# cmhungsteve/TA3N

Measured on NVIDIA H100. Metric: video-clips/sec fwd+bwd (B=256,T=5,D=2048), higher is better.
Workload: dtype tf32x3

## Files before the change

ta3n_b200/csrc/gemm_wgmma.cuh:

```cuda
#pragma once

#include <cuda.h>
#include <stdlib.h>

#include <algorithm>
#include <cmath>
#include <functional>
#include <map>
#include <tuple>

#include "seg_gemm.cuh"

namespace ta3n {

constexpr int TC_BM = 128, TC_BN = 128, TC_BK = 32;
constexpr int TC_THREADS = 288;
constexpr int TC_CONSUMER_WARPS = 8;
constexpr int TC_A_BYTES = TC_BM * TC_BK * 4;
constexpr int TC_B_BYTES = TC_BN * TC_BK * 4;
constexpr int TC_STAGE_BYTES = TC_A_BYTES + TC_B_BYTES;
constexpr int TC_STAGES = 4;
constexpr int tc_smem_bytes(int stages) { return stages * TC_STAGE_BYTES + 1024; }
constexpr int TC_ACC_LD = TC_BN + 4;
constexpr int TC_ACC_BYTES = TC_BM * TC_ACC_LD * 4;
static_assert(TC_ACC_BYTES <= TC_STAGES * TC_STAGE_BYTES, "the per-launch kernel reuses its operand ring");
#ifndef TA3N_MAX_MAPS
#define TA3N_MAX_MAPS 64
#endif
constexpr int kMaxMaps = TA3N_MAX_MAPS;

struct alignas(64) TcMaps {
  CUtensorMap m[kMaxMaps];
};
struct TcSegMaps {
  unsigned char a[kMaxSegs];
  unsigned char b[kMaxSegs];
};

__device__ __forceinline__ uint32_t smem_u32(const void* p) { return (uint32_t)__cvta_generic_to_shared(p); }

__device__ __forceinline__ void mbar_init(uint64_t* bar, uint32_t count) {
  asm volatile("mbarrier.init.shared::cta.b64 [%0], %1;" ::"r"(smem_u32(bar)), "r"(count) : "memory");
}
__device__ __forceinline__ void mbar_expect_tx(uint64_t* bar, uint32_t bytes) {
  asm volatile("mbarrier.arrive.expect_tx.shared::cta.b64 _, [%0], %1;" ::"r"(smem_u32(bar)), "r"(bytes) : "memory");
}
__device__ __forceinline__ void mbar_wait(uint64_t* bar, uint32_t parity) {
  const uint32_t addr = smem_u32(bar);
  uint32_t done;
  do {
    asm volatile(
        "{\n\t.reg .pred p;\n\t"
        "mbarrier.try_wait.parity.shared::cta.b64 p, [%1], %2;\n\t"
        "selp.u32 %0, 1, 0, p;\n\t}"
        : "=r"(done)
        : "r"(addr), "r"(parity)
        : "memory");
  } while (!done);
}
__device__ __forceinline__ void mbar_arrive(uint64_t* bar) {
  asm volatile("mbarrier.arrive.shared::cta.b64 _, [%0];" ::"r"(smem_u32(bar)) : "memory");
}
__device__ __forceinline__ void fence_barrier_init() { asm volatile("fence.mbarrier_init.release.cluster;" ::: "memory"); }
__device__ __forceinline__ void fence_proxy_async() { asm volatile("fence.proxy.async.shared::cta;" ::: "memory"); }
__device__ __forceinline__ void consumer_sync() { asm volatile("bar.sync 1, 256;" ::: "memory"); }

__device__ __forceinline__ void tma_load_2d(void* smem_dst, const CUtensorMap* map, uint64_t* bar, int c0, int c1) {
  asm volatile(
      "cp.async.bulk.tensor.2d.shared::cluster.global.mbarrier::complete_tx::bytes [%0], [%1, {%3, %4}], [%2];"
      ::"r"(smem_u32(smem_dst)), "l"(map), "r"(smem_u32(bar)), "r"(c0), "r"(c1)
      : "memory");
// ... 86 lines not shown
  for (int i = 0; i < 4; ++i) r[i] = lds4(base + mnmaj_chunk(4 * kq + i, mq));
}
__device__ __forceinline__ void tc_prep_store(const uint32_t base, const int t, const float4 (&r)[4]) {
  int mq, kq;
  tc_prep_blk(t, &mq, &kq);
#pragma unroll
  for (int i = 0; i < 4; ++i)
    sts4(base + kmaj_chunk(4 * mq + i, kq), make_float4(f4_at(r[0], i), f4_at(r[1], i), f4_at(r[2], i), f4_at(r[3], i)));
}
__device__ __forceinline__ void tc_prep_stage(const uint32_t a_base, const uint32_t b_base, const bool a_kmaj,
                                              const bool b_kmaj) {
  if (a_kmaj && b_kmaj) return;
  const int t = threadIdx.x;
  float4 ra[4], rb[4];
  if (!a_kmaj) tc_prep_load(a_base, t, ra);
  if (!b_kmaj) tc_prep_load(b_base, t, rb);
  consumer_sync();
  if (!a_kmaj) tc_prep_store(a_base, t, ra);
  if (!b_kmaj) tc_prep_store(b_base, t, rb);
  fence_proxy_async();
  consumer_sync();
}

__device__ __forceinline__ void tc_store_acc(float* acc, const float (&d)[64], const int t) {
  const int lane = t & 31;
  const int row0 = (t >> 7) * 64 + ((t >> 5) & 3) * 16 + (lane >> 2);
#pragma unroll
  for (int j = 0; j < 16; ++j)
#pragma unroll
    for (int h = 0; h < 2; ++h)
      *reinterpret_cast<float2*>(acc + (row0 + 8 * h) * TC_ACC_LD + 8 * j + 2 * (lane & 3)) =
          make_float2(d[4 * j + 2 * h], d[4 * j + 2 * h + 1]);
}
__device__ __forceinline__ void acc_ld_32(const float* acc, int row, int col0, float* v) {
  const float* p = acc + row * TC_ACC_LD + col0;
#pragma unroll
  for (int j = 0; j < 32; j += 4) {
    const float4 q = *reinterpret_cast<const float4*>(p + j);
    v[j] = q.x;
    v[j + 1] = q.y;
    v[j + 2] = q.z;
    v[j + 3] = q.w;
  }
}

struct TcShared {
  uint64_t full_bar[4];
  uint64_t empty_bar[4];
};

template <int STAGES>
__device__ __forceinline__ void tc_pipe_init(TcShared* sh) {
  for (int s = 0; s < STAGES; ++s) {
    mbar_init(&sh->full_bar[s], 1);
    mbar_init(&sh->empty_bar[s], TC_CONSUMER_WARPS);
  }
  fence_barrier_init();
}

enum : int { TILE_FINAL = 0, TILE_PARTIAL = 1 };

template <int STAGES, int STAGE_BYTES = TC_STAGE_BYTES>
__device__ __forceinline__ void tc_produce(const TileCtx& ctx, const CUtensorMap* __restrict__ maps, const bool a_kmaj,
                                           const bool b_kmaj, const int pad_flags, const int m0, const int n0,
                                           const int c_begin, const int n_iter, uint8_t* smem, TcShared* sh,
                                           const uint32_t slabs) {
  const Group& g = ctx.g;
  int seg = 0, k0 = 0;
  {
    int skip = c_begin;
    while (seg < g.seg_count) {
      const int nch = (ctx.seg[seg].len + TC_BK - 1) / TC_BK;
      if (skip < nch) {
        k0 = skip * TC_BK;
        break;
      }
      skip -= nch;
      ++seg;
// ... 35 lines not shown

template <int STAGES>
__device__ __forceinline__ void tc_consume(const bool a_kmaj, const bool b_kmaj, const int n_iter, uint8_t* smem,
                                           TcShared* sh, float (&d)[64]) {
  const int wg = threadIdx.x >> 7, lane = threadIdx.x & 31;
#pragma unroll
  for (int j = 0; j < 64; ++j) d[j] = 0.f;
  int prev = -1;
  for (int it = 0; it < n_iter; ++it) {
    const uint32_t gl = (uint32_t)it;
    const int stage = (int)(gl % STAGES);
    mbar_wait(&sh->full_bar[stage], (gl / STAGES) & 1u);
    const uint32_t a_base = smem_u32(smem + stage * TC_STAGE_BYTES);
    const uint32_t b_base = a_base + TC_A_BYTES;
    tc_prep_stage(a_base, b_base, a_kmaj, b_kmaj);
    wgmma_fence();
#pragma unroll
    for (int ks = 0; ks < TC_BK / 8; ++ks) wgmma_tf32(d, wgmma_desc(a_base + wg * 64 * 128, ks), wgmma_desc(b_base, ks));
    wgmma_commit();
    wgmma_wait<1>();
    if (prev >= 0) {
      __syncwarp();
      if (lane == 0) mbar_arrive(&sh->empty_bar[prev]);
    }
    prev = stage;
  }
  wgmma_wait<0>();
  if (prev >= 0) {
    __syncwarp();
    if (lane == 0) mbar_arrive(&sh->empty_bar[prev]);
  }
}

template <int kEpiWarps>
__device__ __forceinline__ void tc_epilogue(const TileCtx& ctx, const int m0, const int n0, const int split,
                                            const int n_iter, const int mode, const float* acc, const int ew) {
  const int lane = threadIdx.x & 31;
  const int lq = ew & 3;
  const Group e = ctx.g;
  const int m = m0 + lq * 32 + lane;
  const bool split_out = mode == TILE_PARTIAL;
  float* const obase = split_out ? e.partial + (size_t)split * e.M * e.N : e.C;
  const int ldo = split_out ? e.N : e.ldc;
  constexpr int kColChunks = (TC_BN / 32) * 4 / kEpiWarps;
  const int c0 = (ew / 4) * kColChunks;
#pragma unroll 1
  for (int c = c0; c < c0 + kColChunks; ++c) {
    float v[32];
    if (n_iter > 0) {
      acc_ld_32(acc, lq * 32 + lane, c * 32, v);
    } else {
#pragma unroll
      for (int j = 0; j < 32; ++j) v[j] = 0.f;
    }
    const int nb = n0 + c * 32;
    if (m < e.M && nb < e.N) {
      float* orow = obase + (size_t)m * ldo + nb;
      const int nvalid = min(32, e.N - nb);
      if (!split_out) {
        TA3N_EPI_DISPATCH(e.flags, { epilogue_row32<EPI_F>(e, m, nb, nvalid, v); })
      }
      if (nb + 32 <= e.N && ((reinterpret_cast<uintptr_t>(orow) & 15u) == 0)) {
#pragma unroll
        for (int j = 0; j < 32; j += 4)
          *reinterpret_cast<float4*>(orow + j) = make_float4(v[j], v[j + 1], v[j + 2], v[j + 3]);
      } else {
#pragma unroll
        for (int j = 0; j < 32; ++j)
          if (nb + j < e.N) orow[j] = v[j];
      }
    }
  }
}

__device__ __forceinline__ void tc_chunk_range(const TileCtx& ctx, int split, int* c_begin, int* n_iter) {
  const Group& g = ctx.g;
  int total_chunks = 0;
  for (int s = 0; s < g.seg_count; ++s) total_chunks += (ctx.seg[s].len + TC_BK - 1) / TC_BK;
  const int cps = (total_chunks + g.ksplit - 1) / g.ksplit;
  *c_begin = split * cps;
  *n_iter = max(0, min(total_chunks, *c_begin + cps) - *c_begin);
}

__device__ __forceinline__ void tc_decode(const TileCtx& ctx, const int tile, int* split, int* m0, int* n0) {
  const Group& g = ctx.g;
  int local = tile - g.tile_begin;
  const int per_split = g.tiles_m * g.tiles_n;
  *split = local / per_split;
  local -= *split * per_split;
  *m0 = (local / g.tiles_n) * TC_BM;
  *n0 = (local % g.tiles_n) * TC_BN;
}

template <bool A_KMAJ, bool B_KMAJ>
__global__ void __launch_bounds__(TC_THREADS, 1)
seg_gemm_tc_kernel(const __grid_constant__ GemmTable tab, const __grid_constant__ TcMaps maps,
                   const __grid_constant__ TcSegMaps segmaps, const int first_wave) {
  extern __shared__ uint8_t tc_smem_raw[];
  __shared__ __align__(8) TcShared sh;
  uint8_t* smem = reinterpret_cast<uint8_t*>((reinterpret_cast<uintptr_t>(tc_smem_raw) + 1023) & ~uintptr_t(1023));
  const int warp = threadIdx.x >> 5, lane = threadIdx.x & 31;

  __shared__ TileCtx ctx;
  int tile = blockIdx.x;
  if (tile >= first_wave) tile = tab.total_tiles - 1 - (tile - first_wave);
  load_tile_ctx(tab, tile, &ctx, segmaps.a, segmaps.b);
  int split, m0, n0, c_begin, n_iter;
  tc_decode(ctx, tile, &split, &m0, &n0);
  tc_chunk_range(ctx, split, &c_begin, &n_iter);

  if (warp == TC_CONSUMER_WARPS && lane == 0) tc_pipe_init<TC_STAGES>(&sh);
  __syncthreads();
  pdl_wait();

  const int mode = ctx.g.ksplit > 1 ? TILE_PARTIAL : TILE_FINAL;
  if (warp == TC_CONSUMER_WARPS) {
    if (lane == 0 && n_iter > 0)
      tc_produce<TC_STAGES>(ctx, maps.m, A_KMAJ, B_KMAJ, tab.pad_, m0, n0, c_begin, n_iter, smem, &sh, 0u);
  } else {
    float d[64];
    tc_consume<TC_STAGES>(A_KMAJ, B_KMAJ, n_iter, smem, &sh, d);
    consumer_sync();
    float* acc = reinterpret_cast<float*>(smem);
    tc_store_acc(acc, d, threadIdx.x);
    consumer_sync();
    tc_epilogue<TC_CONSUMER_WARPS>(ctx, m0, n0, split, n_iter, mode, acc, warp);
  }
}

constexpr int X3_THREADS = 384;
constexpr int X3_SPLIT_WARPS = 3;
constexpr int X3_SPLIT_THREADS = 32 * X3_SPLIT_WARPS;
constexpr int X3_PRODUCER_REGS = 40, X3_CONSUMER_REGS = 232;
static_assert(128 * X3_PRODUCER_REGS + 256 * X3_CONSUMER_REGS <= X3_THREADS * 168,
              "setmaxnreg budget exceeds the registers of one CTA");
constexpr int X3_STAGES = 4;
constexpr int X3_STAGE_BYTES = TC_STAGE_BYTES + TC_B_BYTES;
constexpr int X3_CHUNK = 8;
static_assert(X3_CHUNK % 2 == 0, "the A fragment register sets alternate by slab within a chunk");
constexpr int x3_smem_bytes() { return X3_STAGES * X3_STAGE_BYTES + 1024; }

constexpr int kX3MaxCtas = 144;
constexpr int kX3MaxTasks = 1024;
struct X3Sched {
  int listed;
  unsigned short off[kX3MaxCtas + 1];
  unsigned short task[kX3MaxTasks];
};
static_assert(sizeof(GemmTable) + sizeof(TcMaps) + sizeof(TcSegMaps) + sizeof(X3Sched) + 256 <= 32764,
              "kernel parameters of the precise kernel exceed the 32 KB limit");

struct X3Slot {
  TileCtx ctx;
  int split, m0, n0, c_begin, n_iter;
};
constexpr int X3_SLOT_READERS = TC_CONSUMER_WARPS + 3;

__device__ __forceinline__ int x3_task(const X3Sched& sched, const int k) {
  return sched.listed ? (int)sched.task[sched.off[blockIdx.x] + k] : (int)(blockIdx.x + k * gridDim.x);
// ... 176 lines not shown
        }
      } else {
        x0 = epilogue_t<F>(g, m, n, x0);
        if (two) x1 = epilogue_t<F>(g, m, n + 1, x1);
      }
      x3_st2(C + (size_t)m * ldc + n, x0, x1, vec, two);
    }
  }
}

__device__ __forceinline__ void x3_finish(const X3Slot& sl, const float (&v)[64]) {
  const Group& g = sl.ctx.g;
  const int warp = threadIdx.x >> 5, lane = threadIdx.x & 31;
  const int m0 = sl.m0 + (warp >> 2) * 64 + (warp & 3) * 16 + (lane >> 2), n0 = sl.n0 + 2 * (lane & 3);
  if (g.ksplit > 1) {
    const int M = g.M, N = g.N;
    float* const part = g.partial + (size_t)sl.split * M * N;
    const bool vec = (N % 2) == 0;
#pragma unroll
    for (int h = 0; h < 2; ++h)
#pragma unroll
      for (int j = 0; j < 16; ++j) {
        const int m = m0 + 8 * h, n = n0 + 8 * j;
        if (m < M && n < N) x3_st2(part + (size_t)m * N + n, v[4 * j + 2 * h], v[4 * j + 2 * h + 1], vec, n + 1 < N);
      }
    return;
  }
  TA3N_EPI_DISPATCH(g.flags, { x3_epilogue<EPI_F>(g, m0, n0, v); })
}

template <bool A_KMAJ, bool B_KMAJ>
__global__ void __launch_bounds__(X3_THREADS, 1)
seg_gemm_tc_x3_kernel(const __grid_constant__ GemmTable tab, const __grid_constant__ TcMaps maps,
                      const __grid_constant__ TcSegMaps segmaps, const __grid_constant__ X3Sched sched) {
  extern __shared__ uint8_t tc_smem_raw[];
  __shared__ __align__(8) TcShared sh;
  __shared__ __align__(8) uint64_t ready_bar[X3_STAGES];
  __shared__ __align__(8) uint64_t slot_full[2], slot_empty[2];
  __shared__ X3Slot slots[2];
  uint8_t* smem = reinterpret_cast<uint8_t*>((reinterpret_cast<uintptr_t>(tc_smem_raw) + 1023) & ~uintptr_t(1023));
  const int warp = threadIdx.x >> 5, lane = threadIdx.x & 31;
  const int n_tasks = sched.listed ? sched.off[blockIdx.x + 1] - sched.off[blockIdx.x]
                                   : (tab.total_tiles - (int)blockIdx.x + (int)gridDim.x - 1) / (int)gridDim.x;

  if (warp == TC_CONSUMER_WARPS) {
    if (lane == 0) {
      for (int s = 0; s < X3_STAGES; ++s) mbar_init(&ready_bar[s], X3_SPLIT_WARPS);
      for (int s = 0; s < 2; ++s) {
        mbar_init(&slot_full[s], 1);
        mbar_init(&slot_empty[s], X3_SLOT_READERS);
      }
      tc_pipe_init<X3_STAGES>(&sh);
    }
    __syncwarp();
    x3_stage(tab, segmaps, x3_task(sched, 0), &slots[0]);
    if (lane == 0) mbar_arrive(&slot_full[0]);
  }
  __syncthreads();
  pdl_wait();

  if (warp >= TC_CONSUMER_WARPS) {
    setmaxnreg_dec<X3_PRODUCER_REGS>();
    uint32_t slabs = 0;
    if (warp == TC_CONSUMER_WARPS) {
      for (int k = 0; k < n_tasks; ++k) {
        const int s = k & 1;
        if (k > 0) {
          mbar_wait(&slot_empty[s], ((uint32_t)(k >> 1) & 1u) ^ 1u);
          x3_stage(tab, segmaps, x3_task(sched, k), &slots[s]);
          if (lane == 0) mbar_arrive(&slot_full[s]);
        }
        const X3Slot& sl = slots[s];
        if (lane == 0 && sl.n_iter > 0)
          tc_produce<X3_STAGES, X3_STAGE_BYTES>(sl.ctx, maps.m, A_KMAJ, B_KMAJ, tab.pad_, sl.m0, sl.n0, sl.c_begin,
                                                sl.n_iter, smem, &sh, slabs);
        __syncwarp();
        slabs += (uint32_t)sl.n_iter;
      }
    } else {
      const int t = threadIdx.x - 32 * (TC_CONSUMER_WARPS + 1);
      for (int k = 0; k < n_tasks; ++k) {
        const int s = k & 1;
        mbar_wait(&slot_full[s], (uint32_t)(k >> 1) & 1u);
        const int n_iter = slots[s].n_iter;
        __syncwarp();
        if (lane == 0) mbar_arrive(&slot_empty[s]);
        for (int it = 0; it < n_iter; ++it) {
          const uint32_t gl = slabs + (uint32_t)it;
          const int stage = (int)(gl % X3_STAGES);
          mbar_wait(&sh.full_bar[stage], (gl / X3_STAGES) & 1u);
          const uint32_t b_raw = smem_u32(smem + stage * X3_STAGE_BYTES) + TC_A_BYTES;
          x3_split_b<B_KMAJ>(b_raw, b_raw + TC_B_BYTES, t);
          fence_proxy_async();
          __syncwarp();
          if (lane == 0) mbar_arrive(&ready_bar[stage]);
        }
        slabs += (uint32_t)n_iter;
      }
    }
  } else {
    setmaxnreg_inc<X3_CONSUMER_REGS>();
    const int r0 = (warp >> 2) * 64 + (warp & 3) * 16 + (lane >> 2);
    const uint32_t off0 = x3_a_thread_off<A_KMAJ>(r0, lane & 3), off1 = x3_a_thread_off<A_KMAJ>(r0 + 8, lane & 3);
    uint32_t slabs = 0;
    for (int k = 0; k < n_tasks; ++k) {
      const int s = k & 1;
      mbar_wait(&slot_full[s], (uint32_t)(k >> 1) & 1u);
      const int n_iter = slots[s].n_iter;
      float d[64], sum[64];
#pragma unroll
      for (int j = 0; j < 64; ++j) d[j] = sum[j] = 0.f;
      uint32_t hi[2][16], lo[2][16];
      int prev = -1;
      for (int c0 = 0; c0 < n_iter; c0 += X3_CHUNK) {
        const int c1 = min(n_iter, c0 + X3_CHUNK);
        for (int it = c0; it < c1; it += 2) {
          x3_consume_slab<A_KMAJ>(slabs + (uint32_t)it, smem, &sh, ready_bar, off0, off1, hi[0], lo[0], d, prev);
          if (it + 1 < c1)
            x3_consume_slab<A_KMAJ>(slabs + (uint32_t)(it + 1), smem, &sh, ready_bar, off0, off1, hi[1], lo[1], d, prev);
        }
        wgmma_wait<0>();
        __syncwarp();
        if (lane == 0) mbar_arrive(&sh.empty_bar[prev]);
        prev = -1;
#pragma unroll
        for (int j = 0; j < 64; ++j) {
          sum[j] += d[j];
          d[j] = 0.f;
        }
      }
      slabs += (uint32_t)n_iter;
      x3_finish(slots[s], sum);
      __syncwarp();
      if (lane == 0) mbar_arrive(&slot_empty[s]);
    }
  }
}

typedef CUresult (*PFN_encodeTiled)(CUtensorMap*, CUtensorMapDataType, cuuint32_t, void*, const cuuint64_t*,
                                    const cuuint64_t*, const cuuint32_t*, const cuuint32_t*, CUtensorMapInterleave,
                                    CUtensorMapSwizzle, CUtensorMapL2promotion, CUtensorMapFloatOOBfill);

inline PFN_encodeTiled encode_fn() {
  static PFN_encodeTiled fn = []() -> PFN_encodeTiled {
    void* p = nullptr;
    cudaDriverEntryPointQueryResult q;
    if (cudaGetDriverEntryPoint("cuTensorMapEncodeTiled", &p, cudaEnableDefault, &q) != cudaSuccess) return nullptr;
    if (q != cudaDriverEntryPointSuccess) return nullptr;
    return reinterpret_cast<PFN_encodeTiled>(p);
  }();
  return fn;
}

struct DeviceInfo {
  int sm_count = 0;
  bool configured[4] = {false, false, false, false};
  bool x3_configured[4] = {false, false, false, false};
  bool eval_configured = false;
};
inline std::mutex& device_mu() {
  static std::mutex mu;
  return mu;
}
inline DeviceInfo* device_info() {
  static std::map<int, DeviceInfo> devs;
  int dev = 0;
  if (cudaGetDevice(&dev) != cudaSuccess) return nullptr;
  DeviceInfo& d = devs[dev];
// ... 65 lines not shown
inline bool tc_group_ok(const GemmPlan& plan, const Group& g) {
  if (plan.load_flags != 0) return false;
  if ((long)g.M * g.N < 64L * 64L) return false;
  if (g.seg_count > kMaxSegs) return false;
  std::map<MapKey, int> maps;
  for (int i = 0; i < g.seg_count; ++i) {
    const Seg& s = plan.segs[g.seg_begin + i];
    if (!tc_operand_ok(s.A, s.lda) || !tc_operand_ok(s.B, s.ldb) || s.len <= 0) return false;
    MapKey ka, kb;
    tc_seg_keys(s, g, plan.a_kmaj, plan.b_kmaj, false, false, &ka, &kb);
    maps[ka] = maps[kb] = 0;
  }
  return (int)maps.size() <= kMaxMaps;
}

template <bool A_KMAJ, bool B_KMAJ>
inline int tc_launch_one(const GemmTable& tab, const TcMaps& maps, const TcSegMaps& sm, cudaStream_t stream,
                         const char* label) {
  constexpr int slot = (A_KMAJ ? 0 : 1) + (B_KMAJ ? 0 : 2);
  int first_wave = 132;
  {
    std::lock_guard<std::mutex> lock(device_mu());
    DeviceInfo* d = device_info();
    if (!d) return fail(TA3N_ERR_CUDA, "cudaGetDevice failed");
    if (!d->configured[slot]) {
      TA3N_CUDA(cudaFuncSetAttribute(seg_gemm_tc_kernel<A_KMAJ, B_KMAJ>, cudaFuncAttributeMaxDynamicSharedMemorySize,
                                     tc_smem_bytes(TC_STAGES)));
      d->configured[slot] = true;
    }
    first_wave = d->sm_count;
  }
  pre_launch(label, stream);
  launch_kernel(seg_gemm_tc_kernel<A_KMAJ, B_KMAJ>, tab.total_tiles, TC_THREADS, tc_smem_bytes(TC_STAGES), stream, tab,
                maps, sm, first_wave);
  return after_launch();
}

template <bool A_KMAJ, bool B_KMAJ>
inline int tc_launch_x3(const GemmTable& tab, const TcMaps& maps, const TcSegMaps& sm, const X3Sched& sched, int grid,
                        cudaStream_t stream, const char* label) {
  constexpr int slot = (A_KMAJ ? 0 : 1) + (B_KMAJ ? 0 : 2);
  {
    std::lock_guard<std::mutex> lock(device_mu());
    DeviceInfo* d = device_info();
    if (!d) return fail(TA3N_ERR_CUDA, "cudaGetDevice failed");
    if (!d->x3_configured[slot]) {
      TA3N_CUDA(cudaFuncSetAttribute(seg_gemm_tc_x3_kernel<A_KMAJ, B_KMAJ>, cudaFuncAttributeMaxDynamicSharedMemorySize,
                                     x3_smem_bytes()));
      d->x3_configured[slot] = true;
    }
  }
  pre_launch(label, stream);
  launch_kernel(seg_gemm_tc_x3_kernel<A_KMAJ, B_KMAJ>, grid, X3_THREADS, x3_smem_bytes(), stream, tab, maps, sm, sched);
  return after_launch();
}

inline GemmPlan sub_plan(const GemmPlan& plan, const std::vector<int>& idx) {
  GemmPlan out;
  out.a_kmaj = plan.a_kmaj;
  out.b_kmaj = plan.b_kmaj;
  out.load_flags = plan.load_flags;
  out.label = plan.label;
  for (int i : idx) {
    Group g = plan.groups[i];
    const int b = g.seg_begin;
    g.seg_begin = (int)out.segs.size();
    for (int k = 0; k < g.seg_count; ++k) out.segs.push_back(plan.segs[b + k]);
    out.groups.push_back(g);
  }
  return out;
}

inline void tc_rank3_flags(const GemmPlan& plan, bool* a3d, bool* b3d) {
  *a3d = !plan.a_kmaj;
  *b3d = !plan.b_kmaj;
  for (const Group& g : plan.groups) {
    if (g.M % 32 != 0) *a3d = false;
    if (g.N % 32 != 0) *b3d = false;
  }
}

inline double x3_makespan(const GemmPlan& plan, const std::vector<int>& ks, int sms,
                          std::vector<std::vector<std::pair<int, int>>>* assign = nullptr);

inline int x3_schedule(const GemmPlan& plan, size_t g_first, const GemmTable& tab, X3Sched* sched) {
  const int ctas = std::min(device_sm_count(), kX3MaxCtas);
// ... 264 lines not shown
```

ta3n_b200/csrc/seg_gemm.cuh:

```cuda
#pragma once

#include <vector>

#include "common.cuh"

namespace ta3n {

#ifndef TA3N_MAX_GROUPS
#define TA3N_MAX_GROUPS 48
#endif
#ifndef TA3N_MAX_SEGS
#define TA3N_MAX_SEGS 128
#endif
constexpr int kMaxGroups = TA3N_MAX_GROUPS;
constexpr int kMaxSegs = TA3N_MAX_SEGS;

enum : int {
  EPI_BIAS = 1,
  EPI_RELU = 2,
  EPI_DROP_MASK = 4,
  EPI_DROP_RNG = 8,
  EPI_ADDROW = 16,
  EPI_GATE = 32,
  EPI_ACCUM = 64,
// ... 64 lines not shown
__device__ __forceinline__ float epilogue_t(const Group& g, int m, int n, float acc) {
  const int f = (F >= 0) ? F : g.flags;
  float v = (g.alpha_dev ? g.alpha * __ldg(g.alpha_dev) : g.alpha) * acc;
  if (f & EPI_BIAS) v += g.bias[n];
  if (f & EPI_RELU) v = fmaxf(v, 0.0f);
  float dropf = 1.0f;
  if (f & EPI_DROP_MASK) dropf = g.keep[(size_t)m * g.ldkeep + n] ? g.drop_scale : 0.0f;
  if (f & EPI_DROP_RNG) {
    uint64_t step = g.step_dev ? *g.step_dev : 0ull;
    dropf = rng_keep(g.seed, step, g.rng_offset + (uint64_t)m * (uint64_t)g.N + (uint64_t)n, g.drop_p) ? g.drop_scale : 0.0f;
  }
  if ((f & (EPI_DROP_MASK | EPI_DROP_RNG)) && !(f & EPI_DROP_LATE)) v = dropf != 0.0f ? v * dropf : 0.0f;
  if (f & EPI_ADDROW) {
    float rs = g.rowscale ? g.rowscale[(size_t)m * g.rs_stride] + g.rs_bias : 1.0f;
    v += rs * g.add[(size_t)m * g.ldadd + n];
  }
  if ((f & (EPI_DROP_MASK | EPI_DROP_RNG)) && (f & EPI_DROP_LATE)) v = dropf != 0.0f ? v * dropf : 0.0f;
  if (f & EPI_GATE) v = g.gate[(size_t)m * g.ldgate + n] > 0.0f ? v : 0.0f;
  if (f & EPI_ACCUM) v += g.C[(size_t)m * g.ldc + n];
  if (f & EPI_DPRE) v = g.gate[(size_t)m * g.ldgate + n] > 0.0f ? v * g.drop_scale : 0.0f;
  if (f & EPI_MULTI) {
#pragma unroll
    for (int q = 0; q < 3; ++q)
      if (q < g.n_multi)
        g.multi_out[q][(size_t)m * g.ldmulti + n] = g.multi_gate[q][(size_t)m * g.ldmulti + n] > 0.0f ? v : 0.0f;
  }
  return v;
}

__device__ __forceinline__ float apply_epilogue(const Group& g, int m, int n, float acc) {
  return epilogue_t<-1>(g, m, n, acc);
}

__device__ __forceinline__ void load_row32(const float* p, int nvalid, float (&r)[32]) {
  if (nvalid >= 32 && (reinterpret_cast<uintptr_t>(p) & 15u) == 0) {
#pragma unroll
    for (int j = 0; j < 32; j += 4) {
      const float4 t = __ldcg(reinterpret_cast<const float4*>(p + j));
      r[j] = t.x;
      r[j + 1] = t.y;
      r[j + 2] = t.z;
      r[j + 3] = t.w;
    }
  } else {
#pragma unroll
    for (int j = 0; j < 32; ++j) r[j] = j < nvalid ? __ldcg(p + j) : 0.f;
  }
}

__device__ __forceinline__ void drop_row32(const Group& g, const int f, int m, int nb, int nvalid, float (&v)[32]) {
  if (f & EPI_DROP_MASK) {
    const uint8_t* k = g.keep + (size_t)m * g.ldkeep + nb;
#pragma unroll
    for (int j = 0; j < 32; ++j)
      if (j < nvalid) v[j] = k[j] ? v[j] * g.drop_scale : 0.0f;
  }
  if (f & EPI_DROP_RNG) {
    const uint64_t step = g.step_dev ? *g.step_dev : 0ull;
    const uint64_t base = g.rng_offset + (uint64_t)m * (uint64_t)g.N + (uint64_t)nb;
    if ((base & 3ull) == 0) {
      const uint32_t thr = rng_threshold(g.drop_p);
#pragma unroll
      for (int j = 0; j < 32; j += 4) {
        const uint64_t hsh = rng_hash4(g.seed, step, (base + j) >> 2);
#pragma unroll
        for (int i = 0; i < 4; ++i) v[j + i] = rng_keep_bits(hsh, i, thr) ? v[j + i] * g.drop_scale : 0.0f;
      }
    } else {
#pragma unroll
      for (int j = 0; j < 32; ++j) v[j] = rng_keep(g.seed, step, base + j, g.drop_p) ? v[j] * g.drop_scale : 0.0f;
    }
  }
}

__device__ __forceinline__ void epilogue_row32_generic(const Group& g, int m, int nb, int nvalid, float (&v)[32]) {
  const int f = g.flags;
  float aux[32];
  const float alpha = g.alpha_dev ? g.alpha * __ldg(g.alpha_dev) : g.alpha;
#pragma unroll
  for (int j = 0; j < 32; ++j) v[j] *= alpha;
  if (f & EPI_BIAS) {
    load_row32(g.bias + nb, nvalid, aux);
#pragma unroll
    for (int j = 0; j < 32; ++j) v[j] += aux[j];
  }
  if (f & EPI_RELU) {
#pragma unroll
    for (int j = 0; j < 32; ++j) v[j] = fmaxf(v[j], 0.0f);
  }
  if ((f & (EPI_DROP_MASK | EPI_DROP_RNG)) && !(f & EPI_DROP_LATE)) drop_row32(g, f, m, nb, nvalid, v);
  if (f & EPI_ADDROW) {
    const float rs = g.rowscale ? __ldcg(g.rowscale + (size_t)m * g.rs_stride) + g.rs_bias : 1.0f;
    load_row32(g.add + (size_t)m * g.ldadd + nb, nvalid, aux);
#pragma unroll
    for (int j = 0; j < 32; ++j) v[j] = fmaf(rs, aux[j], v[j]);
  }
  if ((f & (EPI_DROP_MASK | EPI_DROP_RNG)) && (f & EPI_DROP_LATE)) drop_row32(g, f, m, nb, nvalid, v);
  if (f & EPI_GATE) {
    load_row32(g.gate + (size_t)m * g.ldgate + nb, nvalid, aux);
#pragma unroll
    for (int j = 0; j < 32; ++j) v[j] = aux[j] > 0.0f ? v[j] : 0.0f;
  }
  if (f & EPI_ACCUM) {
    load_row32(g.C + (size_t)m * g.ldc + nb, nvalid, aux);
#pragma unroll
    for (int j = 0; j < 32; ++j) v[j] += aux[j];
  }
  if (f & EPI_DPRE) {
    load_row32(g.gate + (size_t)m * g.ldgate + nb, nvalid, aux);
#pragma unroll
    for (int j = 0; j < 32; ++j) v[j] = aux[j] > 0.0f ? v[j] * g.drop_scale : 0.0f;
  }
  if (f & EPI_MULTI) {
#pragma unroll
    for (int q = 0; q < 3; ++q) {
      if (q >= g.n_multi) break;
      load_row32(g.multi_gate[q] + (size_t)m * g.ldmulti + nb, nvalid, aux);
      float* o = g.multi_out[q] + (size_t)m * g.ldmulti + nb;
#pragma unroll
      for (int j = 0; j < 32; ++j)
        if (j < nvalid) o[j] = aux[j] > 0.f ? v[j] : 0.f;
    }
  }
}

template <int F>
__device__ __forceinline__ void epilogue_row32(const Group& g, int m, int nb, int nvalid, float (&v)[32]) {
  if (F < 0) {
    epilogue_row32_generic(g, m, nb, nvalid, v);
    return;
  }
  const int f = F;
  float a_bias[32], a_add[32], a_gate[32], a_c[32];
  float rs = 1.0f;
  if (f & EPI_BIAS) load_row32(g.bias + nb, nvalid, a_bias);
  if (f & EPI_ADDROW) {
    if (g.rowscale) rs = __ldcg(g.rowscale + (size_t)m * g.rs_stride) + g.rs_bias;
    load_row32(g.add + (size_t)m * g.ldadd + nb, nvalid, a_add);
  }
  if (f & (EPI_GATE | EPI_DPRE)) load_row32(g.gate + (size_t)m * g.ldgate + nb, nvalid, a_gate);
  if (f & EPI_ACCUM) load_row32(g.C + (size_t)m * g.ldc + nb, nvalid, a_c);
  const float alpha = g.alpha_dev ? g.alpha * __ldg(g.alpha_dev) : g.alpha;
#pragma unroll
  for (int j = 0; j < 32; ++j) v[j] *= alpha;
  if (f & EPI_BIAS) {
#pragma unroll
    for (int j = 0; j < 32; ++j) v[j] += a_bias[j];
  }
  if (f & EPI_RELU) {
#pragma unroll
    for (int j = 0; j < 32; ++j) v[j] = fmaxf(v[j], 0.0f);
  }
  if ((f & (EPI_DROP_MASK | EPI_DROP_RNG)) && !(f & EPI_DROP_LATE)) drop_row32(g, f, m, nb, nvalid, v);
  if (f & EPI_ADDROW) {
#pragma unroll
    for (int j = 0; j < 32; ++j) v[j] = fmaf(rs, a_add[j], v[j]);
  }
  if ((f & (EPI_DROP_MASK | EPI_DROP_RNG)) && (f & EPI_DROP_LATE)) drop_row32(g, f, m, nb, nvalid, v);
  if (f & EPI_GATE) {
#pragma unroll
    for (int j = 0; j < 32; ++j) v[j] = a_gate[j] > 0.0f ? v[j] : 0.0f;
  }
  if (f & EPI_ACCUM) {
#pragma unroll
    for (int j = 0; j < 32; ++j) v[j] += a_c[j];
  }
  if (f & EPI_DPRE) {
#pragma unroll
    for (int j = 0; j < 32; ++j) v[j] = a_gate[j] > 0.0f ? v[j] * g.drop_scale : 0.0f;
  }
  if (f & EPI_MULTI) {
#pragma unroll
    for (int q0 = 0; q0 < 3; q0 += 2) {
      if (q0 >= g.n_multi) break;
      float gq[2][32];
#pragma unroll
      for (int u = 0; u < 2; ++u)
        if (q0 + u < 3 && q0 + u < g.n_multi) load_row32(g.multi_gate[q0 + u < 3 ? q0 + u : 2] + (size_t)m * g.ldmulti + nb, nvalid, gq[u]);
#pragma unroll
      for (int u = 0; u < 2; ++u) {
        if (q0 + u >= 3 || q0 + u >= g.n_multi) break;
        float* o = g.multi_out[q0 + u < 3 ? q0 + u : 2] + (size_t)m * g.ldmulti + nb;
        if (nvalid >= 32 && (reinterpret_cast<uintptr_t>(o) & 15u) == 0) {
#pragma unroll
          for (int j = 0; j < 32; j += 4)
            *reinterpret_cast<float4*>(o + j) = make_float4(gq[u][j] > 0.f ? v[j] : 0.f, gq[u][j + 1] > 0.f ? v[j + 1] : 0.f,
                                                            gq[u][j + 2] > 0.f ? v[j + 2] : 0.f, gq[u][j + 3] > 0.f ? v[j + 3] : 0.f);
        } else {
#pragma unroll
          for (int j = 0; j < 32; ++j)
            if (j < nvalid) o[j] = gq[u][j] > 0.f ? v[j] : 0.f;
        }
      }
    }
  }
}

#define TA3N_EPI_DISPATCH(flags, ...)                                              \
  switch (flags) {                                                                  \
    case 0: { constexpr int EPI_F = 0; __VA_ARGS__; } break;                               \
    case (EPI_BIAS | EPI_RELU): { constexpr int EPI_F = EPI_BIAS | EPI_RELU; __VA_ARGS__; } break; \
    case (EPI_BIAS | EPI_RELU | EPI_DROP_RNG): { constexpr int EPI_F = EPI_BIAS | EPI_RELU | EPI_DROP_RNG; __VA_ARGS__; } break; \
    case EPI_ADDROW: { constexpr int EPI_F = EPI_ADDROW; __VA_ARGS__; } break;              \
    case EPI_ACCUM: { constexpr int EPI_F = EPI_ACCUM; __VA_ARGS__; } break;                \
    case (EPI_ACCUM | EPI_DPRE): { constexpr int EPI_F = EPI_ACCUM | EPI_DPRE; __VA_ARGS__; } break; \
    case (EPI_ADDROW | EPI_DROP_RNG | EPI_DROP_LATE): { constexpr int EPI_F = EPI_ADDROW | EPI_DROP_RNG | EPI_DROP_LATE; __VA_ARGS__; } break; \
    case (EPI_ADDROW | EPI_MULTI): { constexpr int EPI_F = EPI_ADDROW | EPI_MULTI; __VA_ARGS__; } break; \
    default: { constexpr int EPI_F = -1; __VA_ARGS__; } break;                              \
  }

struct SegLite {
  const float* A;
  const float* B;
  int len, lda, ldb;
  unsigned short amap, bmap;
};
constexpr int kCtxMaxSegs = kMaxSegs;

struct TileCtx {
  Group g;
  SegLite seg[kCtxMaxSegs];
  int gi;
};

__device__ __forceinline__ void load_tile_ctx(const GemmTable& tab, int tile, TileCtx* ctx,
                                              const unsigned char* amap, const unsigned char* bmap) {
  if (threadIdx.x < 32) {
    int best = 0;
    for (int i = threadIdx.x; i < tab.n_groups; i += 32)
      if (tile >= tab.g[i].tile_begin) best = max(best, i);
// ... 385 lines not shown
```

ta3n_b200/csrc/ta3n_api.cu:

```cuda
#include "common.cuh"
#include "seg_gemm.cuh"
#include "rowops.cuh"
#include "gemm_wgmma.cuh"
#include "optim.cuh"
#include "step_plan.cuh"
#include "allreduce.cuh"
#include "gather.cuh"
#include "eval.cuh"

#include <functional>

using namespace ta3n;

namespace {

struct RelLayout {
  int T, R, n_rel, n_slots;
  std::vector<int> scale_size, rel_count, rel_begin;
  std::vector<int> rel_scale;
  std::vector<int> slot_begin;
  const int* frames;
};

int parse_table(const ta3n_relation_table* tab, RelLayout* L) {
// ... 165 lines not shown
size_t ta3n_wgrad_defer_workspace_bytes(void) { return splitk_bytes(64) + colsum_bytes((size_t)1 << 18); }

int ta3n_wgrad_defer_flush(void* workspace, size_t workspace_bytes, ta3n_stream_t stream) {
  DeferCtx& d = defer_ctx();
  if (!d.active) return fail(TA3N_ERR_INVALID, "ta3n_wgrad_defer_flush without ta3n_wgrad_defer_begin");
  d.active = false;
  Arena arena(workspace, workspace_bytes);
  int rc = d.cs.run(S(stream), &arena);
  if (rc == TA3N_OK) rc = run_gemm(d.wgrad, S(stream), workspace ? &arena : nullptr);
  d.reset();
  return rc;
}

int ta3n_abi_version(void) { return TA3N_ABI_VERSION; }
const char* ta3n_last_error(void) { return last_error_buf(); }
uint64_t ta3n_launch_count(void) { return launch_counter().load(); }
void ta3n_reset_launch_count(void) { launch_counter().store(0); }
int ta3n_set_gemm_engine(int engine) {
  if (engine != TA3N_GEMM_FP32_SIMT && engine != TA3N_GEMM_TF32_TCGEN05 && engine != TA3N_GEMM_TF32X3_TCGEN05)
    return fail(TA3N_ERR_INVALID, "unknown GEMM engine %d", engine);
  gemm_engine().store(engine);
  return TA3N_OK;
}
int ta3n_get_gemm_engine(void) { return gemm_engine().load(); }

int ta3n_set_forward_scratch(void* scratch, size_t bytes) {
  TA3N_REQUIRE(scratch == nullptr || (reinterpret_cast<uintptr_t>(scratch) & 255u) == 0, "scratch must be 256-byte aligned");
  forward_scratch().ptr = bytes > 0 ? scratch : nullptr;
  forward_scratch().bytes = scratch ? bytes : 0;
  return TA3N_OK;
}

void ta3n_timing_enable(int on) { timing().enabled.store(on != 0); }

size_t ta3n_timing_report(char* buf, size_t buf_bytes) {
  TimingRegistry& t = timing();
  std::vector<TimingRegistry::Rec> recs;
  {
    std::lock_guard<std::mutex> g(t.mu);
    recs.swap(t.recs);
  }
  struct Agg {
    const char* label;
    int count;
    double ms;
  };
  std::vector<Agg> agg;
  for (auto& r : recs) {
    float ms = 0.f;
    if (cudaEventSynchronize(r.b) == cudaSuccess && cudaEventElapsedTime(&ms, r.a, r.b) == cudaSuccess) {
      bool found = false;
      for (auto& a : agg)
        if (strcmp(a.label, r.label) == 0) {
          a.count++;
          a.ms += ms;
          found = true;
          break;
        }
      if (!found) agg.push_back({r.label, 1, (double)ms});
    }
    cudaEventDestroy(r.a);
    cudaEventDestroy(r.b);
  }
  std::string out;
  char line[160];
  for (auto& a : agg) {
// ... 937 lines not shown
```

Baseline: 1.074 million.

## Restructure TC epilogue to lane-contiguous columns and add optional timestamp probes

Rewrites the per-launch tensor-core GEMM epilogue so each lane handles four consecutive columns across rows. The old scheme had each thread own one row and 32 columns. Global stores and epilogue operand loads therefore become coalesced across a warp, and the 32-wide register arrays are dropped in favour of a small batch. The old row32 epilogue helpers are removed. It also adds compile-time-gated globaltimer stamps, inactive by default, for profiling kernel phases.

Measured after the change: 1.108 million (median of 6 runs). 1.03x the previous value.

```diff
diff --git a/ta3n_b200/csrc/gemm_wgmma.cuh b/ta3n_b200/csrc/gemm_wgmma.cuh
--- a/ta3n_b200/csrc/gemm_wgmma.cuh
+++ b/ta3n_b200/csrc/gemm_wgmma.cuh
@@ -37,6 +37,60 @@
   unsigned char b[kMaxSegs];
 };
 
+#ifdef TA3N_STAMPS
+constexpr int kStampSlots = 512, kStampPoints = 6;
+__device__ unsigned long long g_stamps[kStampSlots][2][kStampPoints];
+__device__ unsigned int g_stamp_done[kStampSlots];
+struct StampLog {
+  std::mutex mu;
+  int next = 0;
+  const char* label[kStampSlots] = {};
+  bool captured[kStampSlots] = {};
+};
+inline StampLog& stamp_log() {
+  static StampLog l;
+  return l;
+}
+inline int stamp_slot(const char* label, cudaStream_t stream) {
+  StampLog& l = stamp_log();
+  std::lock_guard<std::mutex> g(l.mu);
+  const int s = l.next;
+  l.next = (l.next + 1) % kStampSlots;
+  cudaStreamCaptureStatus cs = cudaStreamCaptureStatusNone;
+  cudaStreamIsCapturing(stream, &cs);
+  l.label[s] = label;
+  l.captured[s] = cs == cudaStreamCaptureStatusActive;
+  return s;
+}
+__device__ __forceinline__ unsigned long long stamp_now() {
+  unsigned long long t;
+  asm volatile("mov.u64 %0, %%globaltimer;" : "=l"(t)::"memory");
+  return t;
+}
+__device__ __forceinline__ void stamp_finish(const int slot, const unsigned long long (&t)[kStampPoints]) {
+  if (blockIdx.x == 0)
+    for (int i = 0; i < kStampPoints; ++i) g_stamps[slot][0][i] = t[i];
+  __threadfence();
+  if (atomicAdd(&g_stamp_done[slot], 1u) == gridDim.x - 1) {
+    for (int i = 0; i < kStampPoints; ++i) g_stamps[slot][1][i] = t[i];
+    g_stamp_done[slot] = 0;
+  }
+}
+#define TA3N_STAMP_PARAM , const int stamp_slot_
+#define TA3N_STAMP_ARG(label, stream) , stamp_slot(label, stream)
+#define TA3N_STAMP_DECL unsigned long long stamps_[kStampPoints] = {}
+#define TA3N_STAMP(i) \
+  if (threadIdx.x == 0) stamps_[i] = stamp_now()
+#define TA3N_STAMP_FINISH() \
+  if (threadIdx.x == 0) stamp_finish(stamp_slot_, stamps_)
+#else
+#define TA3N_STAMP_PARAM
+#define TA3N_STAMP_ARG(label, stream)
+#define TA3N_STAMP_DECL
+#define TA3N_STAMP(i)
+#define TA3N_STAMP_FINISH()
+#endif
+
 __device__ __forceinline__ uint32_t smem_u32(const void* p) { return (uint32_t)__cvta_generic_to_shared(p); }
 
 __device__ __forceinline__ void mbar_init(uint64_t* bar, uint32_t count) {
@@ -189,18 +243,6 @@
       *reinterpret_cast<float2*>(acc + (row0 + 8 * h) * TC_ACC_LD + 8 * j + 2 * (lane & 3)) =
           make_float2(d[4 * j + 2 * h], d[4 * j + 2 * h + 1]);
 }
-__device__ __forceinline__ void acc_ld_32(const float* acc, int row, int col0, float* v) {
-  const float* p = acc + row * TC_ACC_LD + col0;
-#pragma unroll
-  for (int j = 0; j < 32; j += 4) {
-    const float4 q = *reinterpret_cast<const float4*>(p + j);
-    v[j] = q.x;
-    v[j + 1] = q.y;
-    v[j + 2] = q.z;
-    v[j + 3] = q.w;
-  }
-}
-
 struct TcShared {
   uint64_t full_bar[4];
   uint64_t empty_bar[4];
@@ -302,45 +344,64 @@
   }
 }
 
+template <int F, int kEpiWarps>
+__device__ __forceinline__ void tc_epilogue_rows(const Group& g, const int m0, const int n, const int n_iter,
+                                                 float* const obase, const int ldo, const bool raw, const float* acc,
+                                                 const int ew) {
+  constexpr int kRows = TC_BM / kEpiWarps, kBatch = 4;
+  const int M = g.M, N = g.N;
+  const int col = n & (TC_BN - 1);
+#pragma unroll 1
+  for (int r0 = 0; r0 < kRows; r0 += kBatch) {
+    float v[kBatch][4];
+#pragma unroll
+    for (int i = 0; i < kBatch; ++i) {
+      const float4 q = n_iter > 0 ? *reinterpret_cast<const float4*>(acc + (ew + kEpiWarps * (r0 + i)) * TC_ACC_LD + col)
+                                  : make_float4(0.f, 0.f, 0.f, 0.f);
+      v[i][0] = q.x;
+      v[i][1] = q.y;
+      v[i][2] = q.z;
+      v[i][3] = q.w;
+    }
+    if (!raw) {
+#pragma unroll
+      for (int i = 0; i < kBatch; ++i) {
+        const int m = m0 + ew + kEpiWarps * (r0 + i);
+        if (m >= M) continue;
+#pragma unroll
+        for (int j = 0; j < 4; ++j)
+          if (n + j < N) v[i][j] = epilogue_t<F>(g, m, n + j, v[i][j]);
+      }
+    }
+#pragma unroll
+    for (int i = 0; i < kBatch; ++i) {
+      const int m = m0 + ew + kEpiWarps * (r0 + i);
+      if (m >= M) continue;
+      float* o = obase + (size_t)m * ldo + n;
+      if (n + 4 <= N && (reinterpret_cast<uintptr_t>(o) & 15u) == 0) {
+        *reinterpret_cast<float4*>(o) = make_float4(v[i][0], v[i][1], v[i][2], v[i][3]);
+      } else {
+#pragma unroll
+        for (int j = 0; j < 4; ++j)
+          if (n + j < N) o[j] = v[i][j];
+      }
+    }
+  }
+}
+
 template <int kEpiWarps>
 __device__ __forceinline__ void tc_epilogue(const TileCtx& ctx, const int m0, const int n0, const int split,
                                             const int n_iter, const int mode, const float* acc, const int ew) {
-  const int lane = threadIdx.x & 31;
-  const int lq = ew & 3;
-  const Group e = ctx.g;
-  const int m = m0 + lq * 32 + lane;
-  const bool split_out = mode == TILE_PARTIAL;
-  float* const obase = split_out ? e.partial + (size_t)split * e.M * e.N : e.C;
-  const int ldo = split_out ? e.N : e.ldc;
-  constexpr int kColChunks = (TC_BN / 32) * 4 / kEpiWarps;
-  const int c0 = (ew / 4) * kColChunks;
-#pragma unroll 1
-  for (int c = c0; c < c0 + kColChunks; ++c) {
-    float v[32];
-    if (n_iter > 0) {
-      acc_ld_32(acc, lq * 32 + lane, c * 32, v);
-    } else {
-#pragma unroll
-      for (int j = 0; j < 32; ++j) v[j] = 0.f;
-    }
-    const int nb = n0 + c * 32;
-    if (m < e.M && nb < e.N) {
-      float* orow = obase + (size_t)m * ldo + nb;
-      const int nvalid = min(32, e.N - nb);
-      if (!split_out) {
-        TA3N_EPI_DISPATCH(e.flags, { epilogue_row32<EPI_F>(e, m, nb, nvalid, v); })
-      }
-      if (nb + 32 <= e.N && ((reinterpret_cast<uintptr_t>(orow) & 15u) == 0)) {
-#pragma unroll
-        for (int j = 0; j < 32; j += 4)
-          *reinterpret_cast<float4*>(orow + j) = make_float4(v[j], v[j + 1], v[j + 2], v[j + 3]);
-      } else {
-#pragma unroll
-        for (int j = 0; j < 32; ++j)
-          if (nb + j < e.N) orow[j] = v[j];
-      }
-    }
-  }
+  const Group& g = ctx.g;
+  const int n = n0 + 4 * (threadIdx.x & 31);
+  if (n >= g.N) return;
+  const bool raw = mode == TILE_PARTIAL;
+  float* const obase = raw ? g.partial + (size_t)split * g.M * g.N : g.C;
+  const int ldo = raw ? g.N : g.ldc;
+  if (raw)
+    tc_epilogue_rows<0, kEpiWarps>(g, m0, n, n_iter, obase, ldo, true, acc, ew);
+  else
+    TA3N_EPI_DISPATCH(g.flags, { tc_epilogue_rows<EPI_F, kEpiWarps>(g, m0, n, n_iter, obase, ldo, false, acc, ew); })
 }
 
 __device__ __forceinline__ void tc_chunk_range(const TileCtx& ctx, int split, int* c_begin, int* n_iter) {
@@ -365,11 +426,13 @@
 template <bool A_KMAJ, bool B_KMAJ>
 __global__ void __launch_bounds__(TC_THREADS, 1)
 seg_gemm_tc_kernel(const __grid_constant__ GemmTable tab, const __grid_constant__ TcMaps maps,
-                   const __grid_constant__ TcSegMaps segmaps, const int first_wave) {
+                   const __grid_constant__ TcSegMaps segmaps, const int first_wave TA3N_STAMP_PARAM) {
   extern __shared__ uint8_t tc_smem_raw[];
   __shared__ __align__(8) TcShared sh;
   uint8_t* smem = reinterpret_cast<uint8_t*>((reinterpret_cast<uintptr_t>(tc_smem_raw) + 1023) & ~uintptr_t(1023));
   const int warp = threadIdx.x >> 5, lane = threadIdx.x & 31;
+  TA3N_STAMP_DECL;
+  TA3N_STAMP(0);
 
   __shared__ TileCtx ctx;
   int tile = blockIdx.x;
@@ -381,20 +444,32 @@
 
   if (warp == TC_CONSUMER_WARPS && lane == 0) tc_pipe_init<TC_STAGES>(&sh);
   __syncthreads();
+  TA3N_STAMP(1);
   pdl_wait();
+  TA3N_STAMP(2);
 
   const int mode = ctx.g.ksplit > 1 ? TILE_PARTIAL : TILE_FINAL;
   if (warp == TC_CONSUMER_WARPS) {
     if (lane == 0 && n_iter > 0)
       tc_produce<TC_STAGES>(ctx, maps.m, A_KMAJ, B_KMAJ, tab.pad_, m0, n0, c_begin, n_iter, smem, &sh, 0u);
   } else {
+#ifdef TA3N_STAMPS
+    if (threadIdx.x == 0 && n_iter > 0) mbar_wait(&sh.full_bar[0], 0u);
+#endif
+    TA3N_STAMP(3);
     float d[64];
     tc_consume<TC_STAGES>(A_KMAJ, B_KMAJ, n_iter, smem, &sh, d);
+    TA3N_STAMP(4);
     consumer_sync();
     float* acc = reinterpret_cast<float*>(smem);
     tc_store_acc(acc, d, threadIdx.x);
     consumer_sync();
     tc_epilogue<TC_CONSUMER_WARPS>(ctx, m0, n0, split, n_iter, mode, acc, warp);
+#ifdef TA3N_STAMPS
+    consumer_sync();
+#endif
+    TA3N_STAMP(5);
+    TA3N_STAMP_FINISH();
   }
 }
 
@@ -637,7 +712,7 @@
 template <bool A_KMAJ, bool B_KMAJ>
 __global__ void __launch_bounds__(X3_THREADS, 1)
 seg_gemm_tc_x3_kernel(const __grid_constant__ GemmTable tab, const __grid_constant__ TcMaps maps,
-                      const __grid_constant__ TcSegMaps segmaps, const __grid_constant__ X3Sched sched) {
+                      const __grid_constant__ TcSegMaps segmaps, const __grid_constant__ X3Sched sched TA3N_STAMP_PARAM) {
   extern __shared__ uint8_t tc_smem_raw[];
   __shared__ __align__(8) TcShared sh;
   __shared__ __align__(8) uint64_t ready_bar[X3_STAGES];
@@ -645,6 +720,8 @@
   __shared__ X3Slot slots[2];
   uint8_t* smem = reinterpret_cast<uint8_t*>((reinterpret_cast<uintptr_t>(tc_smem_raw) + 1023) & ~uintptr_t(1023));
   const int warp = threadIdx.x >> 5, lane = threadIdx.x & 31;
+  TA3N_STAMP_DECL;
+  TA3N_STAMP(0);
   const int n_tasks = sched.listed ? sched.off[blockIdx.x + 1] - sched.off[blockIdx.x]
                                    : (tab.total_tiles - (int)blockIdx.x + (int)gridDim.x - 1) / (int)gridDim.x;
 
@@ -662,7 +739,9 @@
     if (lane == 0) mbar_arrive(&slot_full[0]);
   }
   __syncthreads();
+  TA3N_STAMP(1);
   pdl_wait();
+  TA3N_STAMP(2);
 
   if (warp >= TC_CONSUMER_WARPS) {
     setmaxnreg_dec<X3_PRODUCER_REGS>();
@@ -708,6 +787,13 @@
     const int r0 = (warp >> 2) * 64 + (warp & 3) * 16 + (lane >> 2);
     const uint32_t off0 = x3_a_thread_off<A_KMAJ>(r0, lane & 3), off1 = x3_a_thread_off<A_KMAJ>(r0 + 8, lane & 3);
     uint32_t slabs = 0;
+#ifdef TA3N_STAMPS
+    if (threadIdx.x == 0) {
+      mbar_wait(&slot_full[0], 0u);
+      if (slots[0].n_iter > 0) mbar_wait(&sh.full_bar[0], 0u);
+    }
+#endif
+    TA3N_STAMP(3);
     for (int k = 0; k < n_tasks; ++k) {
       const int s = k & 1;
       mbar_wait(&slot_full[s], (uint32_t)(k >> 1) & 1u);
@@ -735,10 +821,16 @@
         }
       }
       slabs += (uint32_t)n_iter;
+      TA3N_STAMP(4);
       x3_finish(slots[s], sum);
       __syncwarp();
       if (lane == 0) mbar_arrive(&slot_empty[s]);
     }
+#ifdef TA3N_STAMPS
+    consumer_sync();
+#endif
+    TA3N_STAMP(5);
+    TA3N_STAMP_FINISH();
   }
 }
 
@@ -870,7 +962,7 @@
   }
   pre_launch(label, stream);
   launch_kernel(seg_gemm_tc_kernel<A_KMAJ, B_KMAJ>, tab.total_tiles, TC_THREADS, tc_smem_bytes(TC_STAGES), stream, tab,
-                maps, sm, first_wave);
+                maps, sm, first_wave TA3N_STAMP_ARG(label, stream));
   return after_launch();
 }
 
@@ -889,7 +981,8 @@
     }
   }
   pre_launch(label, stream);
-  launch_kernel(seg_gemm_tc_x3_kernel<A_KMAJ, B_KMAJ>, grid, X3_THREADS, x3_smem_bytes(), stream, tab, maps, sm, sched);
+  launch_kernel(seg_gemm_tc_x3_kernel<A_KMAJ, B_KMAJ>, grid, X3_THREADS, x3_smem_bytes(), stream, tab, maps, sm,
+                sched TA3N_STAMP_ARG(label, stream));
   return after_launch();
 }
 
diff --git a/ta3n_b200/csrc/seg_gemm.cuh b/ta3n_b200/csrc/seg_gemm.cuh
--- a/ta3n_b200/csrc/seg_gemm.cuh
+++ b/ta3n_b200/csrc/seg_gemm.cuh
@@ -120,170 +120,6 @@
   return epilogue_t<-1>(g, m, n, acc);
 }
 
-__device__ __forceinline__ void load_row32(const float* p, int nvalid, float (&r)[32]) {
-  if (nvalid >= 32 && (reinterpret_cast<uintptr_t>(p) & 15u) == 0) {
-#pragma unroll
-    for (int j = 0; j < 32; j += 4) {
-      const float4 t = __ldcg(reinterpret_cast<const float4*>(p + j));
-      r[j] = t.x;
-      r[j + 1] = t.y;
-      r[j + 2] = t.z;
-      r[j + 3] = t.w;
-    }
-  } else {
-#pragma unroll
-    for (int j = 0; j < 32; ++j) r[j] = j < nvalid ? __ldcg(p + j) : 0.f;
-  }
-}
-
-__device__ __forceinline__ void drop_row32(const Group& g, const int f, int m, int nb, int nvalid, float (&v)[32]) {
-  if (f & EPI_DROP_MASK) {
-    const uint8_t* k = g.keep + (size_t)m * g.ldkeep + nb;
-#pragma unroll
-    for (int j = 0; j < 32; ++j)
-      if (j < nvalid) v[j] = k[j] ? v[j] * g.drop_scale : 0.0f;
-  }
-  if (f & EPI_DROP_RNG) {
-    const uint64_t step = g.step_dev ? *g.step_dev : 0ull;
-    const uint64_t base = g.rng_offset + (uint64_t)m * (uint64_t)g.N + (uint64_t)nb;
-    if ((base & 3ull) == 0) {
-      const uint32_t thr = rng_threshold(g.drop_p);
-#pragma unroll
-      for (int j = 0; j < 32; j += 4) {
-        const uint64_t hsh = rng_hash4(g.seed, step, (base + j) >> 2);
-#pragma unroll
-        for (int i = 0; i < 4; ++i) v[j + i] = rng_keep_bits(hsh, i, thr) ? v[j + i] * g.drop_scale : 0.0f;
-      }
-    } else {
-#pragma unroll
-      for (int j = 0; j < 32; ++j) v[j] = rng_keep(g.seed, step, base + j, g.drop_p) ? v[j] * g.drop_scale : 0.0f;
-    }
-  }
-}
-
-__device__ __forceinline__ void epilogue_row32_generic(const Group& g, int m, int nb, int nvalid, float (&v)[32]) {
-  const int f = g.flags;
-  float aux[32];
-  const float alpha = g.alpha_dev ? g.alpha * __ldg(g.alpha_dev) : g.alpha;
-#pragma unroll
-  for (int j = 0; j < 32; ++j) v[j] *= alpha;
-  if (f & EPI_BIAS) {
-    load_row32(g.bias + nb, nvalid, aux);
-#pragma unroll
-    for (int j = 0; j < 32; ++j) v[j] += aux[j];
-  }
-  if (f & EPI_RELU) {
-#pragma unroll
-    for (int j = 0; j < 32; ++j) v[j] = fmaxf(v[j], 0.0f);
-  }
-  if ((f & (EPI_DROP_MASK | EPI_DROP_RNG)) && !(f & EPI_DROP_LATE)) drop_row32(g, f, m, nb, nvalid, v);
-  if (f & EPI_ADDROW) {
-    const float rs = g.rowscale ? __ldcg(g.rowscale + (size_t)m * g.rs_stride) + g.rs_bias : 1.0f;
-    load_row32(g.add + (size_t)m * g.ldadd + nb, nvalid, aux);
-#pragma unroll
-    for (int j = 0; j < 32; ++j) v[j] = fmaf(rs, aux[j], v[j]);
-  }
-  if ((f & (EPI_DROP_MASK | EPI_DROP_RNG)) && (f & EPI_DROP_LATE)) drop_row32(g, f, m, nb, nvalid, v);
-  if (f & EPI_GATE) {
-    load_row32(g.gate + (size_t)m * g.ldgate + nb, nvalid, aux);
-#pragma unroll
-    for (int j = 0; j < 32; ++j) v[j] = aux[j] > 0.0f ? v[j] : 0.0f;
-  }
-  if (f & EPI_ACCUM) {
-    load_row32(g.C + (size_t)m * g.ldc + nb, nvalid, aux);
-#pragma unroll
-    for (int j = 0; j < 32; ++j) v[j] += aux[j];
-  }
-  if (f & EPI_DPRE) {
-    load_row32(g.gate + (size_t)m * g.ldgate + nb, nvalid, aux);
-#pragma unroll
-    for (int j = 0; j < 32; ++j) v[j] = aux[j] > 0.0f ? v[j] * g.drop_scale : 0.0f;
-  }
-  if (f & EPI_MULTI) {
-#pragma unroll
-    for (int q = 0; q < 3; ++q) {
-      if (q >= g.n_multi) break;
-      load_row32(g.multi_gate[q] + (size_t)m * g.ldmulti + nb, nvalid, aux);
-      float* o = g.multi_out[q] + (size_t)m * g.ldmulti + nb;
-#pragma unroll
-      for (int j = 0; j < 32; ++j)
-        if (j < nvalid) o[j] = aux[j] > 0.f ? v[j] : 0.f;
-    }
-  }
-}
-
-template <int F>
-__device__ __forceinline__ void epilogue_row32(const Group& g, int m, int nb, int nvalid, float (&v)[32]) {
-  if (F < 0) {
-    epilogue_row32_generic(g, m, nb, nvalid, v);
-    return;
-  }
-  const int f = F;
-  float a_bias[32], a_add[32], a_gate[32], a_c[32];
-  float rs = 1.0f;
-  if (f & EPI_BIAS) load_row32(g.bias + nb, nvalid, a_bias);
-  if (f & EPI_ADDROW) {
-    if (g.rowscale) rs = __ldcg(g.rowscale + (size_t)m * g.rs_stride) + g.rs_bias;
-    load_row32(g.add + (size_t)m * g.ldadd + nb, nvalid, a_add);
-  }
-  if (f & (EPI_GATE | EPI_DPRE)) load_row32(g.gate + (size_t)m * g.ldgate + nb, nvalid, a_gate);
-  if (f & EPI_ACCUM) load_row32(g.C + (size_t)m * g.ldc + nb, nvalid, a_c);
-  const float alpha = g.alpha_dev ? g.alpha * __ldg(g.alpha_dev) : g.alpha;
-#pragma unroll
-  for (int j = 0; j < 32; ++j) v[j] *= alpha;
-  if (f & EPI_BIAS) {
-#pragma unroll
-    for (int j = 0; j < 32; ++j) v[j] += a_bias[j];
-  }
-  if (f & EPI_RELU) {
-#pragma unroll
-    for (int j = 0; j < 32; ++j) v[j] = fmaxf(v[j], 0.0f);
-  }
-  if ((f & (EPI_DROP_MASK | EPI_DROP_RNG)) && !(f & EPI_DROP_LATE)) drop_row32(g, f, m, nb, nvalid, v);
-  if (f & EPI_ADDROW) {
-#pragma unroll
-    for (int j = 0; j < 32; ++j) v[j] = fmaf(rs, a_add[j], v[j]);
-  }
-  if ((f & (EPI_DROP_MASK | EPI_DROP_RNG)) && (f & EPI_DROP_LATE)) drop_row32(g, f, m, nb, nvalid, v);
-  if (f & EPI_GATE) {
-#pragma unroll
-    for (int j = 0; j < 32; ++j) v[j] = a_gate[j] > 0.0f ? v[j] : 0.0f;
-  }
-  if (f & EPI_ACCUM) {
-#pragma unroll
-    for (int j = 0; j < 32; ++j) v[j] += a_c[j];
-  }
-  if (f & EPI_DPRE) {
-#pragma unroll
-    for (int j = 0; j < 32; ++j) v[j] = a_gate[j] > 0.0f ? v[j] * g.drop_scale : 0.0f;
-  }
-  if (f & EPI_MULTI) {
-#pragma unroll
-    for (int q0 = 0; q0 < 3; q0 += 2) {
-      if (q0 >= g.n_multi) break;
-      float gq[2][32];
-#pragma unroll
-      for (int u = 0; u < 2; ++u)
-        if (q0 + u < 3 && q0 + u < g.n_multi) load_row32(g.multi_gate[q0 + u < 3 ? q0 + u : 2] + (size_t)m * g.ldmulti + nb, nvalid, gq[u]);
-#pragma unroll
-      for (int u = 0; u < 2; ++u) {
-        if (q0 + u >= 3 || q0 + u >= g.n_multi) break;
-        float* o = g.multi_out[q0 + u < 3 ? q0 + u : 2] + (size_t)m * g.ldmulti + nb;
-        if (nvalid >= 32 && (reinterpret_cast<uintptr_t>(o) & 15u) == 0) {
-#pragma unroll
-          for (int j = 0; j < 32; j += 4)
-            *reinterpret_cast<float4*>(o + j) = make_float4(gq[u][j] > 0.f ? v[j] : 0.f, gq[u][j + 1] > 0.f ? v[j + 1] : 0.f,
-                                                            gq[u][j + 2] > 0.f ? v[j + 2] : 0.f, gq[u][j + 3] > 0.f ? v[j + 3] : 0.f);
-        } else {
-#pragma unroll
-          for (int j = 0; j < 32; ++j)
-            if (j < nvalid) o[j] = gq[u][j] > 0.f ? v[j] : 0.f;
-        }
-      }
-    }
-  }
-}
-
 #define TA3N_EPI_DISPATCH(flags, ...)                                              \
   switch (flags) {                                                                  \
     case 0: { constexpr int EPI_F = 0; __VA_ARGS__; } break;                               \
diff --git a/ta3n_b200/csrc/ta3n_api.cu b/ta3n_b200/csrc/ta3n_api.cu
--- a/ta3n_b200/csrc/ta3n_api.cu
+++ b/ta3n_b200/csrc/ta3n_api.cu
@@ -221,6 +221,28 @@
 }
 
 void ta3n_timing_enable(int on) { timing().enabled.store(on != 0); }
+
+#ifdef TA3N_STAMPS
+void ta3n_stamps_reset(void) {
+  std::lock_guard<std::mutex> g(stamp_log().mu);
+  stamp_log().next = 0;
+  for (int i = 0; i < kStampSlots; ++i) stamp_log().label[i] = nullptr;
+}
+int ta3n_stamps_read(unsigned long long* out, int n, char* buf, size_t buf_bytes) {
+  n = std::min(n, kStampSlots);
+  TA3N_CUDA(cudaDeviceSynchronize());
+  TA3N_CUDA(cudaMemcpyFromSymbol(out, g_stamps, sizeof(unsigned long long) * 2 * kStampPoints * n));
+  std::string s;
+  {
+    StampLog& l = stamp_log();
+    std::lock_guard<std::mutex> g(l.mu);
+    for (int i = 0; i < n; ++i)
+      if (l.label[i]) s += std::to_string(i) + " " + (l.captured[i] ? "1 " : "0 ") + l.label[i] + "\n";
+  }
+  snprintf(buf, buf_bytes, "%s", s.c_str());
+  return TA3N_OK;
+}
+#endif
 
 size_t ta3n_timing_report(char* buf, size_t buf_bytes) {
   TimingRegistry& t = timing();
```
